# sh-lee97/grafx

Hardware: AMD Instinct MI355X
Metric: audio samples/sec (rendered output frames of the 32-channel console graph, all GPUs) (higher is better)
Workload: dtype f32; 1 GPU; BASELINE configs[3]: 32-channel mixing console, 111 nodes / 142 edges, ParametricEqualizer(6) + Compressor(iir) + STFTMaskedNoiseReverb + bus sums; batch_per_gpu=256, global_batch=256, audio_len=131072, channels=2, fsm_fir_len=4001, iir_len=16383, ir_len=60001, mode=forward render, reference-exact lengths (even L+N-1), parallelism=batch-shard x1, console_variant=headline, launch=eager render loop

## Files before the change

### grafx_amd/_lib.py

```python
import ctypes
import os

from .build import LIB

i64, f32p, vp, sz = ctypes.c_int64, ctypes.c_void_p, ctypes.c_void_p, ctypes.c_size_t


class RowMap(ctypes.Structure):
    _fields_ = [("inner", i64), ("stride_outer", i64), ("stride_inner", i64), ("stride_ch", i64)]


SIGNATURES = {
    "gfx_abi_version": (ctypes.c_int, []),
    "gfx_device_info": (ctypes.c_int, [ctypes.POINTER(ctypes.c_int), ctypes.POINTER(sz)]),
    "gfx_fftconv_nparts": (i64, [i64]),
    "gfx_fir_spectrum_bytes": (sz, [i64, i64]),
    "gfx_fftconv_workspace_bytes": (sz, [i64, i64, i64, i64, i64, i64]),
    "gfx_fir_spectrum_f32": (ctypes.c_int, [f32p, f32p, i64, vp, i64, i64, vp]),
    "gfx_fftconv_f32": (ctypes.c_int, [f32p, RowMap, vp, f32p, RowMap, i64, i64, i64, i64, i64, i64, i64, vp, sz, vp]),
    "gfx_fftconv_ex_f32": (ctypes.c_int, [f32p, RowMap, vp, i64, i64, f32p, RowMap, f32p, RowMap, i64, i64, i64, i64, i64, i64, i64, vp, sz, vp]),
    "gfx_fftconv_sched_f32": (ctypes.c_int, [f32p, RowMap, vp, i64, i64, f32p, RowMap, f32p, RowMap, i64, i64, i64, i64, i64, i64, i64, vp, sz, ctypes.c_int, vp]),
    "gfx_fftconv_rowmax_f32": (ctypes.c_int, [f32p, RowMap, vp, i64, i64, f32p, RowMap, f32p, RowMap, i64, i64, i64, i64, i64, i64, i64, vp, sz, vp, ctypes.POINTER(ctypes.c_int), vp]),
    "gfx_fftconv_state_f32": (ctypes.c_int, [f32p, RowMap, vp, i64, f32p, RowMap, f32p, f32p, i64, i64, i64, i64, i64, vp, sz,
                                             ctypes.c_int, vp]),
# ... 28 lines not shown
    "gfx_onepole_energy_f32": (ctypes.c_int, [f32p, RowMap, i64, f32p, f32p, i64, i64, i64, i64, ctypes.c_int, vp, vp]),
    "gfx_odd_alias_pair_rows_max_f32": (ctypes.c_int, [f32p, f32p, RowMap, i64, i64, i64, i64, i64, i64, vp, vp, sz, vp, vp]),
    "gfx_odd_alias_pair_precise_plan_bytes": (sz, [i64]),
    "gfx_odd_alias_pair_precise_workspace_bytes": (sz, [i64, i64]),
    "gfx_odd_alias_pair_precise_plan_f32": (ctypes.c_int, [vp, i64, vp, sz, vp]),
    "gfx_odd_alias_pair_precise_f32": (ctypes.c_int, [f32p, f32p, i64, i64, i64, i64, i64, vp, vp, sz, vp]),
    "gfx_irdft_f32": (ctypes.c_int, [f32p, ctypes.c_int, f32p, i64, i64, i64, i64, f32p, vp]),
    "gfx_rdft_f32": (ctypes.c_int, [f32p, f32p, i64, i64, i64, vp]),
    "gfx_iir_fsm_native": (ctypes.c_int, [i64]),
    "gfx_iir_fsm_plan_bytes": (sz, [i64]),
    "gfx_iir_fsm_plan_f32": (ctypes.c_int, [vp, i64, vp]),
    "gfx_iir_fsm_fir_f32": (ctypes.c_int, [f32p, f32p, vp, f32p, i64, i64, i64, vp]),
    "gfx_iir_fsm_fir_f64c_f32": (ctypes.c_int, [vp, vp, vp, f32p, i64, i64, i64, vp]),
    "gfx_iir_fsm_bwd_f32": (ctypes.c_int, [f32p, f32p, f32p, f32p, f32p, f32p, i64, i64, i64, vp]),
    "gfx_peq_coeffs_f32": (ctypes.c_int, [f32p, f32p, f32p, f32p, f32p, i64, i64, ctypes.c_int, vp]),
    "gfx_peq_coeffs_bwd_f32": (ctypes.c_int, [f32p] * 8 + [i64, i64, ctypes.c_int, vp]),
    "gfx_biquad_coeffs_f32": (ctypes.c_int, [f32p, f32p, f32p, f32p, f32p, f32p, i64, vp]),
    "gfx_dynamics_fused_f32": (ctypes.c_int, [f32p, RowMap, f32p, RowMap, f32p, f32p, f32p, f32p, i64, i64, i64,
                                              ctypes.c_int, i64, ctypes.c_int, ctypes.c_int, vp]),
    "gfx_dynamics_fused_ex_f32": (ctypes.c_int, [f32p, RowMap, f32p, RowMap, f32p, f32p, f32p, f32p, i64, i64, i64, i64,
                                                 ctypes.c_int, i64, ctypes.c_int, ctypes.c_int, vp]),
    "gfx_dynamics_fused_u1_f32": (ctypes.c_int, [f32p, RowMap, f32p, RowMap, f32p, f32p, f32p, f32p, i64, i64, i64, i64,
                                                 ctypes.c_int, i64, ctypes.c_int, ctypes.c_int, f32p, vp]),
    "gfx_dynamics_bwd_u1_f32": (ctypes.c_int, [f32p, RowMap, f32p, RowMap, f32p, f32p, f32p, f32p, i64, i64, i64, i64,
                                               ctypes.c_int, ctypes.c_int, f32p, RowMap, f32p, f32p, f32p, vp]),
    "gfx_dynamics_bwd_u1_ws_f32": (ctypes.c_int, [f32p, RowMap, f32p, RowMap, f32p, f32p, f32p, f32p, i64, i64, i64, i64,
                                                  ctypes.c_int, ctypes.c_int, f32p, RowMap, f32p, f32p, f32p, vp, sz, vp]),
    "gfx_dynamics_bwd_rescan_ws_f32": (ctypes.c_int, [f32p, RowMap, f32p, RowMap, f32p, f32p, f32p, f32p, i64, i64, i64, i64,
                                                      ctypes.c_int, ctypes.c_int, f32p, RowMap, f32p, f32p, f32p, vp, sz, vp]),
    "gfx_stft_f32": (ctypes.c_int, [f32p, f32p, f32p, i64, i64, i64, i64, vp]),
    "gfx_dynamics_ws_bytes": (sz, [i64]),
# ... 94 lines not shown
```

### grafx_amd/csrc/fft_tile.hpp

```cpp
#pragma once
#include <hip/hip_runtime.h>

namespace gfx {

constexpr int TILE_M = 8192;
constexpr int TILE_F = 16384;
constexpr int TILE_T = 256;
constexpr int S1_ROW = 272;
constexpr int S2_ROW = 18;
constexpr int TILE_LDS_F2 = 512 * S2_ROW;
constexpr int TILE_LDS_BYTES = TILE_LDS_F2 * 8;
constexpr int H_SLOTS = 17;
constexpr int H_TILE_F4 = H_SLOTS * TILE_T;

using cx = float __attribute__((ext_vector_type(2)));
using f4v = float __attribute__((ext_vector_type(4)));

__device__ __forceinline__ cx to_cx(float2 a) { return cx{a.x, a.y}; }
__device__ __forceinline__ cx cadd(cx a, cx b) { return a + b; }
__device__ __forceinline__ cx csub(cx a, cx b) { return a - b; }
__device__ __forceinline__ cx cswap(cx a) { return __builtin_shufflevector(a, a, 1, 0); }
__device__ __forceinline__ cx cconj(cx a) { return a * cx{1.0f, -1.0f}; }
__device__ __forceinline__ cx mul_neg_i(cx a) { return cswap(a) * cx{1.0f, -1.0f}; }
__device__ __forceinline__ cx mul_pos_i(cx a) { return cswap(a) * cx{-1.0f, 1.0f}; }
// ... 288 lines not shown
__device__ __forceinline__ void for_each_pair(int t, cx wj, Fn&& fn) {
    if (t != 0) {
#pragma unroll
        for (int k3 = 0; k3 < 16; ++k3) fn(k3, k3, 16 + (15 - k3), mul_w16(wj, k3), false);
    } else {
        const cx one = {1.0f, 0.0f};
        fn(0, 0, 0, one, true);
        fn(8, 8, 8, mul_w16(one, 8), true);
#pragma unroll
        for (int k3 = 1; k3 < 8; ++k3) fn(k3, k3, 16 - k3, mul_w16(one, k3), false);
#pragma unroll
        for (int k3 = 0; k3 < 8; ++k3) fn(9 + k3, 16 + k3, 16 + (15 - k3), tw32<false>(one, 1 + 2 * k3), false);
    }
}

}
```

### grafx_amd/csrc/fftconv.hip

```cpp
#include <hip/hip_runtime.h>

#include <cstdint>
#include <type_traits>

#include "../../include/grafx_amd.h"
#include "fft_tile.hpp"

namespace gfx {

struct ConvGeom {
    int64_t nparts, part_len, O, V, ntiles, hop;
    bool ok;
};

static inline ConvGeom conv_geom(int64_t N, int64_t Lout, int64_t part_len = 0) {
    ConvGeom g;
    g.ok = true;
    if (N <= TILE_M + 1) {
        g.nparts = 1;
        g.part_len = N;
        g.O = (N - 1 + 511) & ~int64_t(511);
        g.ok = part_len == 0;
    } else if (part_len == 0 || part_len == TILE_M) {
        g.part_len = TILE_M;
// ... 188 lines not shown

template <bool REV>
__global__ __launch_bounds__(TILE_T, 2) void hspec_kernel(const float* __restrict__ h, const float* __restrict__ gain,
                                                          int64_t gain_div, float4* __restrict__ Hs, int64_t N,
                                                          int nparts, int64_t part_len, gfx_rowmap_t hmap, int C,
                                                          const float2* __restrict__ twtab) {
    extern __shared__ __attribute__((aligned(16))) cx lds[];
    const int t = threadIdx.x;
    const unsigned b = blockIdx.x;
    const unsigned rc = b / (unsigned)nparts;
    const int p = (int)(b - rc * (unsigned)nparts);
    const int64_t start = (int64_t)p * part_len;
    const int64_t len = min(part_len, N - start);

    TileTw tw;
    cx v[32], w[2][16];
    if (REV) {
        const unsigned r = rc / (unsigned)C;
        load_window_rev(v, h + row_off(hmap, r, (int)(rc - r * (unsigned)C)) + (N - start - len), len, t);
    } else {
        load_window(v, h + (int64_t)rc * N + start, 0, len, t, gain ? gain[rc / (unsigned)gain_div] : 1.0f);
    }
    tile_twiddles(tw, twtab, t);
    tile_forward(v, w, tw, lds, t);

    f4v* out = reinterpret_cast<f4v*>(Hs) + (int64_t)b * H_TILE_F4;
    const float sc = 1.0f / (4.0f * TILE_M);
    for_each_pair(t, tw.base(), [&](int slot, int ia, int ib, cx, bool) {
        cx he, ho;
        pair_split(NAT(w, ia), NAT(w, ib), he, ho);
        out[slot * TILE_T + t] = __builtin_shufflevector(he * sc, ho * sc, 0, 1, 2, 3);
    });
}

__device__ __forceinline__ bool window_live(int64_t s, int64_t L) { return s + TILE_F > 0 && s < L; }

#define FC_STATE 0
#include "fftconv_window_kernels.hpp"
#undef FC_STATE
#define FC_STATE 1
#include "fftconv_window_kernels.hpp"
#undef FC_STATE

__global__ __launch_bounds__(TILE_T, 2) void macinv_kernel(const float2* __restrict__ Zs, const float4* __restrict__ Hs,
                                                           float* __restrict__ y, ConvArgs a, int64_t nwin,
                                                           const float2* __restrict__ twtab,
                                                           uint32_t* __restrict__ rowmax = nullptr) {
// ... 736 lines not shown
```

### grafx_amd/csrc/iir_fsm.hip

```cpp
#include <hip/hip_runtime.h>

#include <cstdint>

#include "../../include/grafx_amd.h"
#include "fft_tile.hpp"

#define NAT(arr, i) arr[(i) >> 4][brev((i) & 15, 4)]

namespace gfx {

constexpr int FSM_MAX_N = 4096;
constexpr int PLAN_CHIRP = TILE_M, PLAN_D = TILE_M + FSM_MAX_N, PLAN_FLOAT2 = PLAN_D + 2 * (FSM_MAX_N / 2 + 4);
static inline bool fsm_pow2(int64_t N) { return N == 8192 || N == 16384; }

__device__ __forceinline__ float2 chirp(int k, int N, float sign) {
    const int r = (int)(((int64_t)k * k) % (2 * (int64_t)N));
    float s, c;
    sincospif((float)r / (float)N, &s, &c);
    return make_float2(c, sign * s);
}

__device__ __forceinline__ void sample_points(int k, int N, float2& d1, float2& d2);

__global__ __launch_bounds__(TILE_T, 2) void bluestein_plan_kernel(float2* __restrict__ plan, int N,
// ... 62 lines not shown
                                                   float2 d1, float2 d2, int k, int N, const double* __restrict__ Bd = nullptr,
                                                   const double* __restrict__ Ad = nullptr) {
    if (Bd) return cascade_response_f64(Bd, Ad, K, k, N);
    float2 H = make_float2(1.0f, 0.0f);
    for (int i = 0; i < K; ++i) {
        const float b0 = B[3 * i], b1 = B[3 * i + 1], b2 = B[3 * i + 2];
        const float a0 = A[3 * i], a1 = A[3 * i + 1], a2 = A[3 * i + 2];
        const float2 num = make_float2((b0 + b1 * d1.x) + b2 * d2.x, (b1 * d1.y) + b2 * d2.y);
        const float2 den = make_float2((a0 + a1 * d1.x) + a2 * d2.x, (a1 * d1.y) + a2 * d2.y);
        const float2 q = cdiv(num, den);
        H = (i == 0) ? q : make_float2(fmaf(H.x, q.x, -H.y * q.y), fmaf(H.x, q.y, H.y * q.x));
    }
    return H;
}

__global__ __launch_bounds__(TILE_T, 2) void iir_fsm_kernel(const float* __restrict__ Bs, const float* __restrict__ As,
                                                            const float2* __restrict__ plan, float* __restrict__ h,
                                                            int K, int N, const float2* __restrict__ twtab,
                                                            const double* __restrict__ Bs64, const double* __restrict__ As64) {
    extern __shared__ __attribute__((aligned(16))) cx lds[];
    const int t = threadIdx.x;
    const int64_t rc = blockIdx.x;
    const float* B = Bs ? Bs + rc * K * 3 : nullptr;
    const float* A = As ? As + rc * K * 3 : nullptr;
    const double* Bd = Bs64 ? Bs64 + rc * K * 3 : nullptr;
    const double* Ad = As64 ? As64 + rc * K * 3 : nullptr;
    const int half = N / 2;
    const bool even = (N & 1) == 0;

    TileTw tw;
    tile_twiddles(tw, twtab, t);
    cx v[32], w[2][16];
#pragma unroll
    for (int a = 0; a < 9; ++a) {
        const int k = t + 256 * a;
        if (k <= half) {
            const float4 d = reinterpret_cast<const float4*>(plan + PLAN_D)[k];
            lds[k] = to_cx(cascade_response(B, A, K, make_float2(d.x, d.y), make_float2(d.z, d.w), k, N, Bd, Ad));
        }
    }
    __syncthreads();
#pragma unroll
    for (int a = 0; a < 32; ++a) {
        const int k = t + 256 * a;
        cx e = {0.0f, 0.0f};
        if (a < 17 && k < N) {
            const bool upper = k > half;
            cx Hk = lds[upper ? N - k : k];
            if (upper) Hk.y = -Hk.y;
            if (k == 0 || (even && k == half)) Hk.y = 0.0f;
            e = cmul(Hk, to_cx(plan[PLAN_CHIRP + k]));
        }
        v[a] = e;
    }
    __syncthreads();
    tile_forward(v, w, tw, lds, t);
#pragma unroll
    for (int q = 0; q < 32; ++q) w[q >> 4][q & 15] = cmul(w[q >> 4][q & 15], reinterpret_cast<const cx*>(plan)[q * TILE_T + t]);
    __syncthreads();
    tile_inverse(w, v, tw, lds, t);
    const float sc = 1.0f / ((float)N * (float)TILE_M);
    float* out = h + rc * N;
#pragma unroll
    for (int a = 0; a < 32; ++a) {
        const int n = t + 256 * a;
        if (n < N) {
            const float2 c = plan[PLAN_CHIRP + n];
            const cx e = v[brev(a, 5)];
            out[n] = (e.x * c.x - e.y * c.y) * sc;
        }
    }
}

__global__ __launch_bounds__(TILE_T, 2) void iir_fsm_pow2_kernel(const float* __restrict__ Bs, const float* __restrict__ As,
                                                                 float* __restrict__ h, int K, int N,
                                                                 const float2* __restrict__ twtab,
                                                                 const double* __restrict__ Bs64,
                                                                 const double* __restrict__ As64) {
    extern __shared__ __attribute__((aligned(16))) cx lds[];
    const int t = threadIdx.x;
    const int64_t rc = blockIdx.x;
    const float* B = Bs ? Bs + rc * K * 3 : nullptr;
    const float* A = As ? As + rc * K * 3 : nullptr;
    const double* Bd = Bs64 ? Bs64 + rc * K * 3 : nullptr;
    const double* Ad = As64 ? As64 + rc * K * 3 : nullptr;
    const int stride = TILE_F / N;
    TileTw tw;
    tile_twiddles(tw, twtab, t);
    cx v[32], w[2][16];
    auto Y = [&](int bin) -> cx {
        if (bin % stride) return cx{0.0f, 0.0f};
        const int k = bin / stride;
        float2 d1, d2;
        sample_points(k, N, d1, d2);
        cx r = to_cx(cascade_response(B, A, K, d1, d2, k, N, Bd, Ad));
        if (k == 0 || k == N / 2) r.y = 0.0f;
        return r;
    };
    for_each_pair(t, tw.base(), [&](int, int ia, int ib, cx, bool self) {
        const int j = (ia >> 4) ? bf_b(t) : bf_a(t);
        const int k = j + 512 * (ia & 15);
        const cx ya = Y(k), yb = (self && k != 0) ? ya : Y(TILE_M - k);
        float sn, cs;
        sincospif((float)k / (float)TILE_M, &sn, &cs);
        const cx ye = (ya + cconj(yb)) * 0.5f;
        const cx yo = cmul((ya - cconj(yb)) * 0.5f, cx{cs, sn});
        cx za, zb;
        pair_merge(ye, yo, za, zb);
        NAT(w, ia) = za;
        if (!self) NAT(w, ib) = zb;
    });
    tile_inverse(w, v, tw, lds, t);
    const float sc = (float)stride / (float)TILE_M;
    float* out = h + rc * N;
#pragma unroll
    for (int a = 0; a < 32; ++a) {
        const int n = 2 * (t + 256 * a);
        const cx e = v[brev(a, 5)] * sc;
        if (n + 1 < N) *reinterpret_cast<float2*>(out + n) = make_float2(e.x, e.y);
    }
}

__global__ void peq_coeffs_kernel(const float* __restrict__ w0, const float* __restrict__ q_inv,
                                  const float* __restrict__ log_gain, float* __restrict__ Bs, float* __restrict__ As,
                                  int64_t n, int K, int shelving) {
    const int64_t i = (int64_t)blockIdx.x * blockDim.x + threadIdx.x;
    if (i >= n * K) return;
    const int band = (int)(i % K);
    const float pi32 = 3.14159274101257324219f;
    const float w = pi32 * (1.0f / (1.0f + expf(-w0[i])));
    const float qi = expf(q_inv[i]);
    const float A = expf(log_gain[i]);
    float sw, cw;
    sincosf(w, &sw, &cw);
    const float alpha = sw * qi * 0.5f;
    float b0, b1, b2, a0, a1, a2;
    const bool low = shelving && band == 0, high = shelving && band == K - 1;
    if (low || high) {
        const float sg = low ? 1.0f : -1.0f;
        const float ap1 = A + 1.0f, am1 = A - 1.0f;
        const float ap1c = ap1 * cw, am1c = am1 * cw;
        const float s = 2.0f * sqrtf(A) * alpha;
        b0 = A * ((ap1 - sg * am1c) + s);
        b1 = sg * 2.0f * A * (am1 - sg * ap1c);
        b2 = A * ((ap1 - sg * am1c) - s);
        a0 = (ap1 + sg * am1c) + s;
        a1 = -sg * 2.0f * (am1 + sg * ap1c);
        a2 = (ap1 + sg * am1c) - s;
    } else {
        const float aA = alpha * A, adA = alpha / A;
        b0 = 1.0f + aA;
        b1 = -2.0f * cw;
        b2 = 1.0f - aA;
        a0 = 1.0f + adA;
        a1 = b1;
        a2 = 1.0f - adA;
    }
    Bs[3 * i] = b0;
    Bs[3 * i + 1] = b1;
    Bs[3 * i + 2] = b2;
    As[3 * i] = a0;
    As[3 * i + 1] = a1;
    As[3 * i + 2] = a2;
}

__global__ void peq_coeffs_bwd_kernel(const float* __restrict__ w0, const float* __restrict__ q_inv,
                                      const float* __restrict__ log_gain, const float* __restrict__ gBs,
                                      const float* __restrict__ gAs, float* __restrict__ gw0, float* __restrict__ gq,
                                      float* __restrict__ glg, int64_t n, int K, int shelving) {
    const int64_t i = (int64_t)blockIdx.x * blockDim.x + threadIdx.x;
    if (i >= n * K) return;
    const int band = (int)(i % K);
    const float pi32 = 3.14159274101257324219f;
    const float sig = 1.0f / (1.0f + expf(-w0[i]));
    const float w = pi32 * sig;
    const float qi = expf(q_inv[i]);
    const float A = expf(log_gain[i]);
    float sw, cw;
// ... 155 lines not shown
int gfx_iir_fsm_fir_f64c_f32(const double* Bs, const double* As, const void* plan, float* h, int64_t RC, int64_t K,
                             int64_t N, void* stream) {
    if (!Bs || !As) return GFX_EINVAL;
    return iir_fsm_fir_launch(nullptr, nullptr, Bs, As, plan, h, RC, K, N, stream);
}

int gfx_peq_coeffs_f32(const float* w0, const float* q_inv, const float* log_gain, float* Bs, float* As, int64_t n,
                       int64_t K, int use_shelving, void* stream) {
    if (!w0 || !q_inv || !log_gain || !Bs || !As || n <= 0 || K <= 0) return GFX_EINVAL;
    const int64_t total = n * K;
    hipLaunchKernelGGL(peq_coeffs_kernel, dim3((unsigned)((total + 255) / 256)), dim3(256), 0, (hipStream_t)stream, w0,
                       q_inv, log_gain, Bs, As, n, (int)K, use_shelving);
    return hipGetLastError() == hipSuccess ? GFX_OK : GFX_ELAUNCH;
}

int gfx_peq_coeffs_bwd_f32(const float* w0, const float* q_inv, const float* log_gain, const float* gBs, const float* gAs,
                           float* gw0, float* gq_inv, float* glog_gain, int64_t n, int64_t K, int use_shelving,
                           void* stream) {
    if (!w0 || !q_inv || !log_gain || !gBs || !gAs || !gw0 || !gq_inv || !glog_gain || n <= 0 || K <= 0) return GFX_EINVAL;
    const int64_t total = n * K;
    hipLaunchKernelGGL(peq_coeffs_bwd_kernel, dim3((unsigned)((total + 255) / 256)), dim3(256), 0, (hipStream_t)stream, w0,
                       q_inv, log_gain, gBs, gAs, gw0, gq_inv, glog_gain, n, (int)K, use_shelving);
    return hipGetLastError() == hipSuccess ? GFX_OK : GFX_ELAUNCH;
}

int gfx_biquad_coeffs_f32(const float* Bin, const float* A1_pre, const float* A2_pre, const float* A0, float* Bs,
                          float* As, int64_t n, void* stream) {
    if (!Bin || !A1_pre || !A2_pre || !Bs || !As || n <= 0) return GFX_EINVAL;
    hipLaunchKernelGGL(biquad_coeffs_kernel, dim3((unsigned)((n + 255) / 256)), dim3(256), 0, (hipStream_t)stream, Bin,
                       A1_pre, A2_pre, A0, Bs, As, n);
// ... 15 lines not shown
```

### grafx_amd/ops.py

```python
import contextvars
import ctypes
import os

import torch

from ._lib import RowMap, check, lib


_PROFILE = contextvars.ContextVar("grafx_amd_profile", default=None)


class profiling:
    def __enter__(self):
        self.record = {}
        self.token = _PROFILE.set(self.record)
        return self.record

    def __exit__(self, *exc):
        _PROFILE.reset(self.token)
        return False


class _timed:
    def __init__(self, name, nbytes):
# ... 532 lines not shown


@_on_device
def peq_coeffs(w0, q_inv, log_gain, use_shelving=True):
    _require_gpu(w0, q_inv, log_gain)
    w0, q_inv, log_gain = w0.contiguous(), q_inv.contiguous(), log_gain.contiguous()
    K = w0.shape[-1]
    n = w0.numel() // K
    Bs = torch.empty((*w0.shape, 3), dtype=torch.float32, device=w0.device)
    As = torch.empty_like(Bs)
    check(lib().gfx_peq_coeffs_f32(_ptr(w0), _ptr(q_inv), _ptr(log_gain), _ptr(Bs), _ptr(As), n, K, int(use_shelving), _stream()),
          "gfx_peq_coeffs_f32")
    return Bs, As


@_on_device
def peq_coeffs_bwd(w0, q_inv, log_gain, gBs, gAs, use_shelving=True):
    _require_gpu(w0, q_inv, log_gain, gBs, gAs)
    w0, q_inv, log_gain = w0.contiguous(), q_inv.contiguous(), log_gain.contiguous()
    _expect(gBs, (*w0.shape, 3), "peq_coeffs_bwd: gBs")
    _expect(gAs, (*w0.shape, 3), "peq_coeffs_bwd: gAs")
    K = w0.shape[-1]
    out = [torch.empty_like(w0) for _ in range(3)]
    pin = _Pin()
    check(lib().gfx_peq_coeffs_bwd_f32(_ptr(w0), _ptr(q_inv), _ptr(log_gain), pin(gBs), pin(gAs),
                                       *(_ptr(o) for o in out), w0.numel() // K, K, int(use_shelving), _stream()),
          "gfx_peq_coeffs_bwd_f32")
    return tuple(out)


# ... 653 lines not shown
```

### grafx_amd/processors/core/iir.py

```python
import torch
import torch.nn as nn

from ... import autograd as diff
from ... import ops
from ...autograd import needs_grad
from ._buffer_io import StreamIO, write_rows
from .convolution import FIRConvolution, check_state, convolve_taps


def map_signal(fn, result):
    return (fn(result[0]), *result[1:]) if isinstance(result, tuple) else fn(result)


class BiquadStream(StreamIO):

    def stream_block(self, x4, out4, carry, **params):
        key = "history" if self.biquad.backend == "fsm" else "state"
        y, carry = self.forward(x4.reshape(-1, *x4.shape[2:]), **params, **{key: carry, "return_" + key: True})
        write_rows(out4, y)
        return carry


class IIRFilter(nn.Module):
    def __init__(self, order=2, backend="fsm", flashfftconv=True, fsm_fir_len=4000,
# ... 134 lines not shown
        if needs_grad(x, Bs, As, history):
            if N <= self.FSM_NATIVE_MAX and Bs.shape[-1] == 3:
                h = diff.FsmFirFn.apply(Bs, As, N, self._plan(Bs.device))
            else:
                h = diff.fsm_fir(Bs, As, N)
            y, zf = diff.convolve(x, h, "causal", final=final, state=check_state(history, x, N, "IIRFilter(backend='fsm')"),
                                  return_state=True)
            if out is not None:
                out.copy_(y.view(out.shape))
                y = out
        else:
            y, zf = convolve_taps(x, ops.fir_spectrum(self._taps(Bs, As)), N, Bs.shape[1], "causal", out=out,
                                  h_rows=shared_rows, state=history, return_state=True)
        return (y, zf) if return_history else y

    def forward(self, input_signal, Bs, As, out=None, tee=None, shared_rows=None, final=False, state=None,
                return_state=False, history=None, return_history=False):
        if self.backend == "fsm" and (state is not None or return_state):
            raise ValueError("IIRFilter(backend='fsm'): the frequency-sampled FIR carries no recursive state; use the "
                             "recursive backends (backend='lfilter' or 'ssm') for block-wise processing")
        if history is not None or return_history:
            if self.backend != "fsm":
                raise ValueError(f"IIRFilter(backend={self.backend!r}): history / return_history carry the input history of the "
                                 "frequency-sampled FIR (backend='fsm'); a recursive backend carries state / return_state")
            return self._process_fsm_block(input_signal, Bs, As, out, tee, shared_rows, final, history, return_history)
        if shared_rows is not None and self.backend != "fsm":
            rows = input_signal.shape[0] * input_signal.shape[1] if input_signal.ndim == 4 else input_signal.shape[0]
            Bs, As = Bs.repeat(rows // shared_rows, 1, 1, 1), As.repeat(rows // shared_rows, 1, 1, 1)
            shared_rows = None
        if self.backend != "fsm":
# ... 22 lines not shown
```

### grafx_amd/processors/eq.py

```python
import torch
import torch.nn as nn

from .. import ops
from .core._buffer_io import BufferIO, Prepared, StreamIO, expand_shared, shared_reps, write_rows
from .core.convolution import convolve, convolve_taps
from .core.fir import ZeroPhaseFilterBankFIR, ZeroPhaseFIR
from .core.geq import GraphicEqualizerBiquad
from .. import autograd as diff
from ..autograd import needs_grad
from .core.iir import BiquadStream, IIRFilter, map_signal
from .core.midside import lr_to_ms, ms_to_lr


class ParametricEqualizer(BufferIO, nn.Module):
    def __init__(self, num_filters=10, processor_channel="mono", use_shelving_filters=True, **backend_kwargs):
        super().__init__()
        self.num_filters = num_filters
        self.use_shelving_filters = use_shelving_filters
        self.biquad = IIRFilter(order=2, **backend_kwargs)
        self.processor_channel = processor_channel
        if processor_channel not in ("mono", "stereo", "midside"):
            raise ValueError(f"Invalid processor_channel: {self.processor_channel}")

    accepts_tee = True
    accepts_shared_params = True
    accepts_strided_rows = True

    def forward(self, input_signals, w0, q_inv, log_gain, _out=None, _tee=None, _shared_rows=None, state=None,
                return_state=False, history=None, return_history=False):
        self._check_bands()
        if needs_grad(input_signals, w0, q_inv, log_gain):
            Bs, As = diff.PeqCoeffsFn.apply(w0, q_inv, log_gain, self.use_shelving_filters)
        else:
            Bs, As = ops.peq_coeffs(w0, q_inv, log_gain, self.use_shelving_filters)
        block = {} if state is None and not return_state else {"state": state, "return_state": return_state}
        if history is not None or return_history:
            block.update(history=history, return_history=return_history)
        if self.processor_channel == "midside":
            y = self.biquad(lr_to_ms(input_signals), Bs, As, shared_rows=_shared_rows, final=True, **block)
            return (ms_to_lr(y[0]), y[1]) if return_state or return_history else ms_to_lr(y)
        return self.biquad(input_signals, Bs, As, out=_out, tee=_tee, shared_rows=_shared_rows, final=True, **block)

    def get_biquad_coefficients_with_shelving_filters(self, cos_w0, alpha, A):
        from .filter import HighShelf, LowShelf, PeakingFilter

        self._check_bands()
        K = self.num_filters
        parts = [LowShelf.get_biquad_coefficients(cos_w0[..., :1], alpha[..., :1], A[..., :1]),
                 PeakingFilter.get_biquad_coefficients(cos_w0[..., 1 : K - 1], alpha[..., 1 : K - 1], A[..., 1 : K - 1]),
                 HighShelf.get_biquad_coefficients(cos_w0[..., K - 1 :], alpha[..., K - 1 :], A[..., K - 1 :])]
        return torch.cat([b for b, _ in parts], -2), torch.cat([a for _, a in parts], -2)

    def _check_bands(self):
        if self.use_shelving_filters and self.num_filters < 2:
            raise RuntimeError(f"split expects non-negative sizes, got [1, {self.num_filters - 2}, 1]: "
                               "shelving filters need num_filters >= 2")

    def prepare(self, w0, q_inv, log_gain, _shared_rows=None):
        self._check_bands()
        if self.processor_channel == "midside" or self.biquad.backend != "fsm" or needs_grad(w0, q_inv, log_gain):
            return None
        Bs, As = ops.peq_coeffs(w0, q_inv, log_gain, self.use_shelving_filters)
        return Prepared(ops.fir_spectrum(self.biquad._taps(Bs, As)), Cf=Bs.shape[1])

    def render_into(self, x4, out4, tee=None, _shared_rows=None, _prepared=None, history=None, return_history=False,
                    **params):
        if history is not None or return_history:
            if _prepared is not None:
                y, zf = convolve_taps(x4, _prepared.tensors[0], self.biquad.fsm_fir_len, _prepared.Cf, "causal", out=out4,
                                      tee=tee, h_rows=_shared_rows, state=history, return_state=True)
            elif self.processor_channel == "midside":
                if tee is not None:
                    tee.copy_(x4)
                y, zf = self.forward(x4, _shared_rows=_shared_rows, history=history, return_history=True, **params)
                y = write_rows(out4, y)
            else:
                y, zf = self.forward(x4, _out=out4, _tee=tee, _shared_rows=_shared_rows, history=history,
                                     return_history=True, **params)
# ... 97 lines not shown
```

### grafx_amd/render/graph.py

```python
import contextlib
import warnings

import torch

from ..data.configs import UTILITY_TYPES
from .core import (
    aggregate_tensor,
    create_signal_buffer,
    expand_tensor_or_tensor_dict,
    flatten_batch_and_node,
    inplace_write_tensor,
    read_tensor_or_tensor_dict,
)


KEEP_SMOOTHER_SCAN = False
PREPARE_MODE = "under_first"

BLOCK_FAN_ADJOINT = True


def _gather_plan(step, device):
    cache = step.__dict__.setdefault("_plans", {})
    key = (device.type, device.index)
# ... 245 lines not shown
                      keep_signal_buffer=True):
    from .. import ops

    squeeze = input_signals.ndim == 3
    x = input_signals.unsqueeze(0) if squeeze else input_signals
    B, n_src, C, L = x.shape
    shared_tree = per_type_parameters if (not squeeze and common_parameters is None) else None
    if not squeeze:
        expanded_tree = None
        if common_parameters is not None:
            common_parameters = expand_tensor_or_tensor_dict(common_parameters, expand=B, dim=0)
    node_dim = 0 if squeeze else 1
    postprocess = None if squeeze else flatten_batch_and_node

    buf = torch.empty(B, render_data.num_nodes, C, L, device=x.device)
    lean = not keep_signal_buffer
    teed = None if lean else _tee_range(render_data, processors, n_src, x.device)
    main = torch.cuda.current_stream(x.device)
    rest = [] if lean else _complement(teed, n_src)
    sources_in_buf = not lean
    side = _side_stream(x.device) if rest else None
    if side is not None:
        side.wait_stream(main)
        with torch.cuda.stream(side):
            for a, b in rest:
                buf[:, a:b].copy_(x[:, a:b], non_blocking=True)
    copied = False
    out_view = None

    def ensure_sources():
        nonlocal sources_in_buf
        if not sources_in_buf:
            buf[:, :n_src].copy_(x)
            sources_in_buf = True

    def stage_parameters(step, proc):
        nonlocal expanded_tree
        extra = {}
        if squeeze:
            params = read_tensor_or_tensor_dict(per_type_parameters[step.node_type], step.parameter_read, dim=0)
        elif shared_tree is not None and getattr(proc, "accepts_shared_params", False):
            params = read_tensor_or_tensor_dict(shared_tree[step.node_type], step.parameter_read, dim=0)
            extra["_shared_rows"] = step.dest_write.idx[1] - step.dest_write.idx[0]
        else:
# ... 18 lines not shown
        prep.wait_stream(main)
        ready = {}
        with torch.cuda.stream(prep):
            for j in todo:
                proc_j = processors[render_data.iter_list[j].node_type]
                extra_j, params_j, common_j = args[j]
                state = proc_j.prepare(**extra_j, **params_j, **common_j)
                if state is None:
                    continue
                for tns in state.tensors:
                    tns.record_stream(main)
                event = torch.cuda.Event()
                event.record(prep)
                ready[j] = (state, event)
        return ready

    prepared = None
    launched = 0
    done = set()

    def run_stage(i, mix_with=None):
        nonlocal copied, prepared, launched
        step = render_data.iter_list[i]
        d0, d1 = step.dest_write.idx
        out_v = buf.narrow(1, d0, d1 - d0)
        plan = _gather_plan(step, x.device)
        node_type = step.node_type
        src_read = step.source_reads[0]
        from_inputs = plan is None and src_read.idx[1] <= n_src
        if side is not None and not from_inputs and not copied and _touches_inputs(src_read, n_src):
# ... 2 lines not shown
        if lean and not from_inputs and _touches_inputs(src_read, n_src):
            ensure_sources()
        if node_type not in processors:
            if plan is None:
                a, b = step.source_reads[0].idx
                out_v.copy_((x if from_inputs else buf).narrow(1, a, b - a))
            else:
                _gather(ops, buf, plan, out_v)
            return False
        if plan is None:
            a, b = step.source_reads[0].idx
            x_view = (x if from_inputs else buf).narrow(1, a, b - a)
        else:
            x_view = _gather(ops, buf, plan, torch.empty(B, plan[2], C, L, device=x.device))
        proc = processors[node_type]
        extra, params, common_i = stage_parameters(step, proc)
        if teed is not None and i == _first_order(render_data):
            a, b = teed
            extra["tee"] = buf.narrow(1, a, b - a)
        if prepared is not None and i in prepared:
            state, event = prepared[i]
            main.wait_event(event)
            extra["_prepared"] = state
        if (aux is not None and plan is None and KEEP_SMOOTHER_SCAN and getattr(proc, "accepts_aux", False)
                and type(proc) in _tape_safe_types()):
            extra["_aux"] = (aux, i)
        mix = None
        if mix_with is not None:
            nxt = render_data.iter_list[mix_with]
            sched = _mix_schedule(step, nxt, x.device)
            if side is not None and not copied and any(r < n_src for r in sched["extra_rows"]):
# ... 646 lines not shown
```

### include/grafx_amd.h

```cpp
#ifndef GRAFX_AMD_H
#define GRAFX_AMD_H

#include <stddef.h>
#include <stdint.h>

#ifdef __cplusplus
extern "C" {
#endif

#define GFX_OK 0
#define GFX_EINVAL -1
#define GFX_ENOSPC -2
#define GFX_ELAUNCH -3

typedef struct {
    int64_t inner;
    int64_t stride_outer;
    int64_t stride_inner;
    int64_t stride_ch;
} gfx_rowmap_t;

int gfx_abi_version(void);
int gfx_device_info(int* n_cu, size_t* lds_bytes);

// ... 92 lines not shown

int gfx_iir_fsm_native(int64_t N);
size_t gfx_iir_fsm_plan_bytes(int64_t N);
int gfx_iir_fsm_plan_f32(void* plan, int64_t N, void* stream);
int gfx_iir_fsm_fir_f32(const float* Bs, const float* As, const void* plan, float* h,
                        int64_t RC, int64_t K, int64_t N, void* stream);
int gfx_iir_fsm_fir_f64c_f32(const double* Bs, const double* As, const void* plan, float* h, int64_t RC, int64_t K,
                             int64_t N, void* stream);
int gfx_iir_fsm_bwd_f32(const float* Bs, const float* As, const float* G, const float* delays, float* gB, float* gA,
                        int64_t RC, int64_t K, int64_t N, void* stream);

int gfx_peq_coeffs_f32(const float* w0, const float* q_inv, const float* log_gain, float* Bs, float* As,
                       int64_t n, int64_t K, int use_shelving, void* stream);
int gfx_biquad_coeffs_f32(const float* Bin, const float* A1_pre, const float* A2_pre, const float* A0,
                          float* Bs, float* As, int64_t n, void* stream);
int gfx_peq_coeffs_bwd_f32(const float* w0, const float* q_inv, const float* log_gain, const float* gBs,
                           const float* gAs, float* gw0, float* gq_inv, float* glog_gain,
                           int64_t n, int64_t K, int use_shelving, void* stream);

int gfx_dynamics_fused_f32(const float* x, gfx_rowmap_t xmap, float* y, gfx_rowmap_t ymap,
                           const float* log_threshold, const float* log_ratio, const float* log_knee,
                           const float* z_alpha, int64_t R, int64_t C, int64_t L, int smoother,
                           int64_t iir_len, int knee, int gate, void* stream);
int gfx_dynamics_fused_ex_f32(const float* x, gfx_rowmap_t xmap, float* y, gfx_rowmap_t ymap,
                              const float* log_threshold, const float* log_ratio, const float* log_knee,
                              const float* z_alpha, int64_t param_rows, int64_t R, int64_t C, int64_t L,
                              int smoother, int64_t iir_len, int knee, int gate, void* stream);
size_t gfx_dynamics_ws_bytes(int64_t param_rows);
size_t gfx_dynamics_ws_bytes_ex(int64_t param_rows, int64_t R, int64_t L);
int gfx_dynamics_fused_ws_f32(const float* x, gfx_rowmap_t xmap, float* y, gfx_rowmap_t ymap,
// ... 155 lines not shown
```

Baseline: 3.366 billion audio samples/s.

## Fuse PEQ coefficient design, FSM impulse response, and filter spectrum into one kernel

Adds a peq_spectra kernel that computes biquad coefficients in LDS, evaluates the frequency-sampled IIR response, and directly produces the tiled FIR spectrum, replacing three separate launches (peq_coeffs, iir_fsm taps, fir_spectrum) and their intermediate global buffers. The render loop also prepares the first-order stage's design before the source copy setup so it can overlap. Shared device helpers are factored out of the existing FSM and spectrum kernels. This adds a large-register, LDS-heavy kernel with one block per row, which could occupy the GPU less efficiently than the separate kernels.

```diff
diff --git a/grafx_amd/_lib.py b/grafx_amd/_lib.py
--- a/grafx_amd/_lib.py
+++ b/grafx_amd/_lib.py
@@ -66,7 +66,8 @@
     "gfx_iir_fsm_fir_f64c_f32": (ctypes.c_int, [vp, vp, vp, f32p, i64, i64, i64, vp]),
     "gfx_iir_fsm_bwd_f32": (ctypes.c_int, [f32p, f32p, f32p, f32p, f32p, f32p, i64, i64, i64, vp]),
     "gfx_peq_coeffs_f32": (ctypes.c_int, [f32p, f32p, f32p, f32p, f32p, i64, i64, ctypes.c_int, vp]),
-    "gfx_peq_coeffs_bwd_f32": (ctypes.c_int, [f32p] * 8 + [i64, i64, ctypes.c_int, vp]),
+    "gfx_peq_spectra_f32": (ctypes.c_int, [f32p, f32p, f32p, RowMap, vp, vp, i64, i64, i64, i64, ctypes.c_int, vp]),
+    "gfx_peq_coeffs_bwd_f32":(ctypes.c_int, [f32p] * 8 + [i64, i64, ctypes.c_int, vp]),
     "gfx_biquad_coeffs_f32": (ctypes.c_int, [f32p, f32p, f32p, f32p, f32p, f32p, i64, vp]),
     "gfx_dynamics_fused_f32": (ctypes.c_int, [f32p, RowMap, f32p, RowMap, f32p, f32p, f32p, f32p, i64, i64, i64,
                                               ctypes.c_int, i64, ctypes.c_int, ctypes.c_int, vp]),
diff --git a/grafx_amd/csrc/fft_tile.hpp b/grafx_amd/csrc/fft_tile.hpp
--- a/grafx_amd/csrc/fft_tile.hpp
+++ b/grafx_amd/csrc/fft_tile.hpp
@@ -326,4 +326,15 @@
     }
 }
 
-}
+__device__ __forceinline__ void tile_filter_spectrum(cx (&v)[32], const TileTw& tw, cx* lds, int t, f4v* __restrict__ out) {
+    cx w[2][16];
+    tile_forward(v, w, tw, lds, t);
+    const float sc = 1.0f / (4.0f * TILE_M);
+    for_each_pair(t, tw.base(), [&](int slot, int ia, int ib, cx, bool) {
+        cx he, ho;
+        pair_split(w[ia >> 4][brev(ia & 15, 4)], w[ib >> 4][brev(ib & 15, 4)], he, ho);
+        out[slot * TILE_T + t] = __builtin_shufflevector(he * sc, ho * sc, 0, 1, 2, 3);
+    });
+}
+
+}
diff --git a/grafx_amd/csrc/fftconv.hip b/grafx_amd/csrc/fftconv.hip
--- a/grafx_amd/csrc/fftconv.hip
+++ b/grafx_amd/csrc/fftconv.hip
@@ -226,7 +226,7 @@
     const int64_t len = min(part_len, N - start);
 
     TileTw tw;
-    cx v[32], w[2][16];
+    cx v[32];
     if (REV) {
         const unsigned r = rc / (unsigned)C;
         load_window_rev(v, h + row_off(hmap, r, (int)(rc - r * (unsigned)C)) + (N - start - len), len, t);
@@ -234,15 +234,7 @@
         load_window(v, h + (int64_t)rc * N + start, 0, len, t, gain ? gain[rc / (unsigned)gain_div] : 1.0f);
     }
     tile_twiddles(tw, twtab, t);
-    tile_forward(v, w, tw, lds, t);
-
-    f4v* out = reinterpret_cast<f4v*>(Hs) + (int64_t)b * H_TILE_F4;
-    const float sc = 1.0f / (4.0f * TILE_M);
-    for_each_pair(t, tw.base(), [&](int slot, int ia, int ib, cx, bool) {
-        cx he, ho;
-        pair_split(NAT(w, ia), NAT(w, ib), he, ho);
-        out[slot * TILE_T + t] = __builtin_shufflevector(he * sc, ho * sc, 0, 1, 2, 3);
-    });
+    tile_filter_spectrum(v, tw, lds, t, reinterpret_cast<f4v*>(Hs) + (int64_t)b * H_TILE_F4);
 }
 
 __device__ __forceinline__ bool window_live(int64_t s, int64_t L) { return s + TILE_F > 0 && s < L; }
diff --git a/grafx_amd/csrc/iir_fsm.hip b/grafx_amd/csrc/iir_fsm.hip
--- a/grafx_amd/csrc/iir_fsm.hip
+++ b/grafx_amd/csrc/iir_fsm.hip
@@ -100,6 +100,49 @@
     return H;
 }
 
+constexpr int FSM_COEF_AT = FSM_MAX_N;
+constexpr int FSM_COEF_MAX_K = 1024;
+__device__ __forceinline__ void fsm_czt(const float* __restrict__ B, const float* __restrict__ A, const double* __restrict__ Bd,
+                                        const double* __restrict__ Ad, const float2* __restrict__ plan, int K, int N,
+                                        const TileTw& tw, cx* lds, int t, cx (&v)[32]) {
+    const int half = N / 2;
+    const bool even = (N & 1) == 0;
+    cx w[2][16];
+#pragma unroll
+    for (int a = 0; a < 9; ++a) {
+        const int k = t + 256 * a;
+        if (k <= half) {
+            const float4 d = reinterpret_cast<const float4*>(plan + PLAN_D)[k];
+            lds[k] = to_cx(cascade_response(B, A, K, make_float2(d.x, d.y), make_float2(d.z, d.w), k, N, Bd, Ad));
+        }
+    }
+    __syncthreads();
+#pragma unroll
+    for (int a = 0; a < 32; ++a) {
+        const int k = t + 256 * a;
+        cx e = {0.0f, 0.0f};
+        if (a < 17 && k < N) {
+            const bool upper = k > half;
+            cx Hk = lds[upper ? N - k : k];
+            if (upper) Hk.y = -Hk.y;
+            if (k == 0 || (even && k == half)) Hk.y = 0.0f;
+            e = cmul(Hk, to_cx(plan[PLAN_CHIRP + k]));
+        }
+        v[a] = e;
+    }
+    __syncthreads();
+    tile_forward(v, w, tw, lds, t);
+#pragma unroll
+    for (int q = 0; q < 32; ++q) w[q >> 4][q & 15] = cmul(w[q >> 4][q & 15], reinterpret_cast<const cx*>(plan)[q * TILE_T + t]);
+    __syncthreads();
+    tile_inverse(w, v, tw, lds, t);
+}
+__device__ __forceinline__ float fsm_tap(const cx (&v)[32], const float2* __restrict__ plan, int a, int n, float sc) {
+    const float2 c = plan[PLAN_CHIRP + n];
+    const cx e = v[brev(a, 5)];
+    return (e.x * c.x - e.y * c.y) * sc;
+}
+
 __global__ __launch_bounds__(TILE_T, 2) void iir_fsm_kernel(const float* __restrict__ Bs, const float* __restrict__ As,
                                                             const float2* __restrict__ plan, float* __restrict__ h,
                                                             int K, int N, const float2* __restrict__ twtab,
@@ -111,69 +154,24 @@
     const float* A = As ? As + rc * K * 3 : nullptr;
     const double* Bd = Bs64 ? Bs64 + rc * K * 3 : nullptr;
     const double* Ad = As64 ? As64 + rc * K * 3 : nullptr;
-    const int half = N / 2;
-    const bool even = (N & 1) == 0;
-
     TileTw tw;
     tile_twiddles(tw, twtab, t);
-    cx v[32], w[2][16];
-#pragma unroll
-    for (int a = 0; a < 9; ++a) {
-        const int k = t + 256 * a;
-        if (k <= half) {
-            const float4 d = reinterpret_cast<const float4*>(plan + PLAN_D)[k];
-            lds[k] = to_cx(cascade_response(B, A, K, make_float2(d.x, d.y), make_float2(d.z, d.w), k, N, Bd, Ad));
-        }
-    }
-    __syncthreads();
-#pragma unroll
-    for (int a = 0; a < 32; ++a) {
-        const int k = t + 256 * a;
-        cx e = {0.0f, 0.0f};
-        if (a < 17 && k < N) {
-            const bool upper = k > half;
-            cx Hk = lds[upper ? N - k : k];
-            if (upper) Hk.y = -Hk.y;
-            if (k == 0 || (even && k == half)) Hk.y = 0.0f;
-            e = cmul(Hk, to_cx(plan[PLAN_CHIRP + k]));
-        }
-        v[a] = e;
-    }
-    __syncthreads();
-    tile_forward(v, w, tw, lds, t);
-#pragma unroll
-    for (int q = 0; q < 32; ++q) w[q >> 4][q & 15] = cmul(w[q >> 4][q & 15], reinterpret_cast<const cx*>(plan)[q * TILE_T + t]);
-    __syncthreads();
-    tile_inverse(w, v, tw, lds, t);
+    cx v[32];
+    fsm_czt(B, A, Bd, Ad, plan, K, N, tw, lds, t, v);
     const float sc = 1.0f / ((float)N * (float)TILE_M);
     float* out = h + rc * N;
 #pragma unroll
     for (int a = 0; a < 32; ++a) {
         const int n = t + 256 * a;
-        if (n < N) {
-            const float2 c = plan[PLAN_CHIRP + n];
-            const cx e = v[brev(a, 5)];
-            out[n] = (e.x * c.x - e.y * c.y) * sc;
-        }
-    }
-}
-
-__global__ __launch_bounds__(TILE_T, 2) void iir_fsm_pow2_kernel(const float* __restrict__ Bs, const float* __restrict__ As,
-                                                                 float* __restrict__ h, int K, int N,
-                                                                 const float2* __restrict__ twtab,
-                                                                 const double* __restrict__ Bs64,
-                                                                 const double* __restrict__ As64) {
-    extern __shared__ __attribute__((aligned(16))) cx lds[];
-    const int t = threadIdx.x;
-    const int64_t rc = blockIdx.x;
-    const float* B = Bs ? Bs + rc * K * 3 : nullptr;
-    const float* A = As ? As + rc * K * 3 : nullptr;
-    const double* Bd = Bs64 ? Bs64 + rc * K * 3 : nullptr;
-    const double* Ad = As64 ? As64 + rc * K * 3 : nullptr;
+        if (n < N) out[n] = fsm_tap(v, plan, a, n, sc);
+    }
+}
+
+__device__ __forceinline__ float fsm_pow2_scale(int N) { return (float)(TILE_F / N) / (float)TILE_M; }
+__device__ __forceinline__ void fsm_pow2_spectrum(const float* __restrict__ B, const float* __restrict__ A,
+                                                  const double* __restrict__ Bd, const double* __restrict__ Ad, int K, int N,
+                                                  const TileTw& tw, int t, cx (&w)[2][16]) {
     const int stride = TILE_F / N;
-    TileTw tw;
-    tile_twiddles(tw, twtab, t);
-    cx v[32], w[2][16];
     auto Y = [&](int bin) -> cx {
         if (bin % stride) return cx{0.0f, 0.0f};
         const int k = bin / stride;
@@ -196,8 +194,26 @@
         NAT(w, ia) = za;
         if (!self) NAT(w, ib) = zb;
     });
+}
+
+__global__ __launch_bounds__(TILE_T, 2) void iir_fsm_pow2_kernel(const float* __restrict__ Bs, const float* __restrict__ As,
+                                                                 float* __restrict__ h, int K, int N,
+                                                                 const float2* __restrict__ twtab,
+                                                                 const double* __restrict__ Bs64,
+                                                                 const double* __restrict__ As64) {
+    extern __shared__ __attribute__((aligned(16))) cx lds[];
+    const int t = threadIdx.x;
+    const int64_t rc = blockIdx.x;
+    const float* B = Bs ? Bs + rc * K * 3 : nullptr;
+    const float* A = As ? As + rc * K * 3 : nullptr;
+    const double* Bd = Bs64 ? Bs64 + rc * K * 3 : nullptr;
+    const double* Ad = As64 ? As64 + rc * K * 3 : nullptr;
+    TileTw tw;
+    tile_twiddles(tw, twtab, t);
+    cx v[32], w[2][16];
+    fsm_pow2_spectrum(B, A, Bd, Ad, K, N, tw, t, w);
     tile_inverse(w, v, tw, lds, t);
-    const float sc = (float)stride / (float)TILE_M;
+    const float sc = fsm_pow2_scale(N);
     float* out = h + rc * N;
 #pragma unroll
     for (int a = 0; a < 32; ++a) {
@@ -207,16 +223,12 @@
     }
 }
 
-__global__ void peq_coeffs_kernel(const float* __restrict__ w0, const float* __restrict__ q_inv,
-                                  const float* __restrict__ log_gain, float* __restrict__ Bs, float* __restrict__ As,
-                                  int64_t n, int K, int shelving) {
-    const int64_t i = (int64_t)blockIdx.x * blockDim.x + threadIdx.x;
-    if (i >= n * K) return;
-    const int band = (int)(i % K);
+__device__ __forceinline__ void peq_section(float w0, float q_inv, float log_gain, int band, int K, int shelving,
+                                            float* __restrict__ Bs, float* __restrict__ As) {
     const float pi32 = 3.14159274101257324219f;
-    const float w = pi32 * (1.0f / (1.0f + expf(-w0[i])));
-    const float qi = expf(q_inv[i]);
-    const float A = expf(log_gain[i]);
+    const float w = pi32 * (1.0f / (1.0f + expf(-w0)));
+    const float qi = expf(q_inv);
+    const float A = expf(log_gain);
     float sw, cw;
     sincosf(w, &sw, &cw);
     const float alpha = sw * qi * 0.5f;
@@ -242,12 +254,80 @@
         a1 = b1;
         a2 = 1.0f - adA;
     }
-    Bs[3 * i] = b0;
-    Bs[3 * i + 1] = b1;
-    Bs[3 * i + 2] = b2;
-    As[3 * i] = a0;
-    As[3 * i + 1] = a1;
-    As[3 * i + 2] = a2;
+    Bs[0] = b0;
+    Bs[1] = b1;
+    Bs[2] = b2;
+    As[0] = a0;
+    As[1] = a1;
+    As[2] = a2;
+}
+
+__global__ void peq_coeffs_kernel(const float* __restrict__ w0, const float* __restrict__ q_inv,
+                                  const float* __restrict__ log_gain, float* __restrict__ Bs, float* __restrict__ As,
+                                  int64_t n, int K, int shelving) {
+    const int64_t i = (int64_t)blockIdx.x * blockDim.x + threadIdx.x;
+    if (i >= n * K) return;
+    peq_section(w0[i], q_inv[i], log_gain[i], (int)(i % K), K, shelving, Bs + 3 * i, As + 3 * i);
+}
+
+template <bool POW2>
+__global__ __launch_bounds__(TILE_T, 2) void peq_spectra_kernel(const float* __restrict__ w0, const float* __restrict__ q_inv,
+                                                                const float* __restrict__ log_gain, gfx_rowmap_t pmap, int Cf,
+                                                                const float2* __restrict__ plan, float4* __restrict__ Hs,
+                                                                int K, int N, int shelving,
+                                                                const float2* __restrict__ twtab) {
+    extern __shared__ __attribute__((aligned(16))) cx lds[];
+    const int t = threadIdx.x;
+    const unsigned rc = blockIdx.x;
+    const unsigned r = rc / (unsigned)Cf;
+    const int c = (int)(rc - r * (unsigned)Cf);
+    const unsigned q = r / (unsigned)pmap.inner;
+    const int64_t p0 = (int64_t)q * pmap.stride_outer + (int64_t)(r - q * (unsigned)pmap.inner) * pmap.stride_inner +
+                       (int64_t)c * pmap.stride_ch;
+    float* B = reinterpret_cast<float*>(lds + FSM_COEF_AT);
+    float* A = B + 3 * K;
+    for (int band = t; band < K; band += TILE_T)
+        peq_section(w0[p0 + band], q_inv[p0 + band], log_gain[p0 + band], band, K, shelving, B + 3 * band, A + 3 * band);
+    __syncthreads();
+
+    TileTw tw;
+    tile_twiddles(tw, twtab, t);
+    cx v[32], h2[32];
+    if (POW2) {
+        cx w[2][16];
+        fsm_pow2_spectrum(B, A, nullptr, nullptr, K, N, tw, t, w);
+        __syncthreads();
+        tile_inverse(w, v, tw, lds, t);
+        const float sc = fsm_pow2_scale(N);
+#pragma unroll
+        for (int a = 0; a < 32; ++a) {
+            const cx e = v[brev(a, 5)] * sc;
+            h2[a] = 2 * (t + 256 * a) + 1 < N ? e : cx{0.0f, 0.0f};
+        }
+    } else {
+        fsm_czt(B, A, nullptr, nullptr, plan, K, N, tw, lds, t, v);
+        const float sc = 1.0f / ((float)N * (float)TILE_M);
+        float* taps = reinterpret_cast<float*>(lds);
+        __syncthreads();
+#pragma unroll
+        for (int a = 0; a < FSM_MAX_N / TILE_T; ++a) {
+            const int n = t + 256 * a;
+            if (n < N) taps[n] = fsm_tap(v, plan, a, n, sc);
+        }
+        __syncthreads();
+#pragma unroll
+        for (int a = 0; a < 32; ++a) {
+            const int n = 2 * (t + 256 * a);
+            cx e = {0.0f, 0.0f};
+            if (a < FSM_MAX_N / 2 / TILE_T) {
+                if (n < N) e.x = taps[n];
+                if (n + 1 < N) e.y = taps[n + 1];
+            }
+            h2[a] = e;
+        }
+    }
+    __syncthreads();
+    tile_filter_spectrum(h2, tw, lds, t, reinterpret_cast<f4v*>(Hs) + (int64_t)rc * H_TILE_F4);
 }
 
 __global__ void peq_coeffs_bwd_kernel(const float* __restrict__ w0, const float* __restrict__ q_inv,
@@ -433,6 +513,21 @@
     return hipGetLastError() == hipSuccess ? GFX_OK : GFX_ELAUNCH;
 }
 
+int gfx_peq_spectra_f32(const float* w0, const float* q_inv, const float* log_gain, gfx_rowmap_t pmap, const void* plan,
+                        void* Hs, int64_t R, int64_t Cf, int64_t K, int64_t N, int use_shelving, void* stream) {
+    if (!w0 || !q_inv || !log_gain || !Hs || R <= 0 || Cf <= 0 || K <= 0 || K > FSM_COEF_MAX_K) return GFX_EINVAL;
+    if (pmap.inner <= 0 || pmap.inner > 0x7fffffffLL || R * Cf > 0x7fffffffLL) return GFX_EINVAL;
+    const bool pow2 = N == TILE_M;
+    if (!pow2 && (N < 1 || N > FSM_MAX_N || !plan)) return GFX_EINVAL;
+    auto* kernel = pow2 ? peq_spectra_kernel<true> : peq_spectra_kernel<false>;
+    if (allow_lds(kernel)) return GFX_ELAUNCH;
+    const float2* tw = tile_twiddle_table((hipStream_t)stream);
+    if (!tw) return GFX_ELAUNCH;
+    hipLaunchKernelGGL(kernel, dim3((unsigned)(R * Cf)), dim3(TILE_T), TILE_LDS_BYTES, (hipStream_t)stream, w0, q_inv,
+                       log_gain, pmap, (int)Cf, (const float2*)plan, (float4*)Hs, (int)K, (int)N, use_shelving, tw);
+    return hipGetLastError() == hipSuccess ? GFX_OK : GFX_ELAUNCH;
+}
+
 int gfx_peq_coeffs_bwd_f32(const float* w0, const float* q_inv, const float* log_gain, const float* gBs, const float* gAs,
                            float* gw0, float* gq_inv, float* glog_gain, int64_t n, int64_t K, int use_shelving,
                            void* stream) {
diff --git a/grafx_amd/ops.py b/grafx_amd/ops.py
--- a/grafx_amd/ops.py
+++ b/grafx_amd/ops.py
@@ -570,6 +570,31 @@
     return Bs, As
 
 
+PEQ_SPECTRA_MAX_K = 1024
+
+
+def peq_spectra_native(N, K):
+    return 1 <= K <= PEQ_SPECTRA_MAX_K and (1 <= N <= 4096 or N == 8192)
+
+
+@_on_device
+def peq_spectra(w0, q_inv, log_gain, N, plan, use_shelving=True):
+    _require_gpu(w0, q_inv, log_gain)
+    if w0.ndim != 3:
+        raise ValueError(f"peq_spectra: expected (R, Cf, K) parameters, got {tuple(w0.shape)}")
+    _expect(q_inv, w0.shape, "peq_spectra: q_inv")
+    _expect(log_gain, w0.shape, "peq_spectra: log_gain")
+    if w0.stride(-1) != 1 or q_inv.stride() != w0.stride() or log_gain.stride() != w0.stride():
+        w0, q_inv, log_gain = w0.contiguous(), q_inv.contiguous(), log_gain.contiguous()
+    R, Cf, K = w0.shape
+    nbytes = lib().gfx_fir_spectrum_bytes_ex(R * Cf, N, 0) if peq_spectra_native(N, K) else 0
+    Hs = torch.empty(nbytes, dtype=torch.uint8, device=w0.device)
+    pmap = RowMap(max(R, 1), 0, w0.stride(0), w0.stride(1))
+    check(lib().gfx_peq_spectra_f32(_ptr(w0), _ptr(q_inv), _ptr(log_gain), pmap, _ptr(plan), _ptr(Hs), R, Cf, K, N,
+                                    int(use_shelving), _stream()), "gfx_peq_spectra_f32")
+    return Hs
+
+
 @_on_device
 def peq_coeffs_bwd(w0, q_inv, log_gain, gBs, gAs, use_shelving=True):
     _require_gpu(w0, q_inv, log_gain, gBs, gAs)
diff --git a/grafx_amd/processors/core/iir.py b/grafx_amd/processors/core/iir.py
--- a/grafx_amd/processors/core/iir.py
+++ b/grafx_amd/processors/core/iir.py
@@ -172,6 +172,14 @@
                                   h_rows=shared_rows, state=history, return_state=True)
         return (y, zf) if return_history else y
 
+    def convolve_spectra(self, x, Hs, Cf, out=None, tee=None, shared_rows=None, history=None, return_history=False):
+        N = self.fsm_fir_len
+        if history is not None or return_history:
+            y, zf = convolve_taps(x, Hs, N, Cf, "causal", out=out, tee=tee, h_rows=shared_rows, state=history,
+                                  return_state=True)
+            return (y, zf) if return_history else y
+        return convolve_taps(x, Hs, N, Cf, "causal", out=out, tee=tee, exact=self.flashfftconv, h_rows=shared_rows)
+
     def forward(self, input_signal, Bs, As, out=None, tee=None, shared_rows=None, final=False, state=None,
                 return_state=False, history=None, return_history=False):
         if self.backend == "fsm" and (state is not None or return_state):
diff --git a/grafx_amd/processors/eq.py b/grafx_amd/processors/eq.py
--- a/grafx_amd/processors/eq.py
+++ b/grafx_amd/processors/eq.py
@@ -29,6 +29,10 @@
     def forward(self, input_signals, w0, q_inv, log_gain, _out=None, _tee=None, _shared_rows=None, state=None,
                 return_state=False, history=None, return_history=False):
         self._check_bands()
+        if state is None and not return_state and self._designs_fused(input_signals, w0, q_inv, log_gain):
+            return self.biquad.convolve_spectra(input_signals, self._design(w0, q_inv, log_gain), w0.shape[1], out=_out,
+                                                tee=_tee, shared_rows=_shared_rows, history=history,
+                                                return_history=return_history)
         if needs_grad(input_signals, w0, q_inv, log_gain):
             Bs, As = diff.PeqCoeffsFn.apply(w0, q_inv, log_gain, self.use_shelving_filters)
         else:
@@ -51,6 +55,18 @@
                  HighShelf.get_biquad_coefficients(cos_w0[..., K - 1 :], alpha[..., K - 1 :], A[..., K - 1 :])]
         return torch.cat([b for b, _ in parts], -2), torch.cat([a for _, a in parts], -2)
 
+    def _designs_fused(self, *tensors):
+        w0 = tensors[-3]
+        return (self.biquad.backend == "fsm" and self.processor_channel != "midside" and not needs_grad(*tensors)
+                and w0.ndim == 3 and ops.peq_spectra_native(self.biquad.fsm_fir_len, w0.shape[-1]))
+
+    def _design(self, w0, q_inv, log_gain):
+        if self._designs_fused(w0, q_inv, log_gain):
+            plan = self.biquad._plan(w0.device) if w0.is_cuda else None
+            return ops.peq_spectra(w0, q_inv, log_gain, self.biquad.fsm_fir_len, plan, self.use_shelving_filters)
+        Bs, As = ops.peq_coeffs(w0, q_inv, log_gain, self.use_shelving_filters)
+        return ops.fir_spectrum(self.biquad._taps(Bs, As))
+
     def _check_bands(self):
         if self.use_shelving_filters and self.num_filters < 2:
             raise RuntimeError(f"split expects non-negative sizes, got [1, {self.num_filters - 2}, 1]: "
@@ -60,8 +76,7 @@
         self._check_bands()
         if self.processor_channel == "midside" or self.biquad.backend != "fsm" or needs_grad(w0, q_inv, log_gain):
             return None
-        Bs, As = ops.peq_coeffs(w0, q_inv, log_gain, self.use_shelving_filters)
-        return Prepared(ops.fir_spectrum(self.biquad._taps(Bs, As)), Cf=Bs.shape[1])
+        return Prepared(self._design(w0, q_inv, log_gain), Cf=w0.shape[1])
 
     def render_into(self, x4, out4, tee=None, _shared_rows=None, _prepared=None, history=None, return_history=False,
                     **params):
diff --git a/grafx_amd/render/graph.py b/grafx_amd/render/graph.py
--- a/grafx_amd/render/graph.py
+++ b/grafx_amd/render/graph.py
@@ -283,20 +283,6 @@
     postprocess = None if squeeze else flatten_batch_and_node
 
     buf = torch.empty(B, render_data.num_nodes, C, L, device=x.device)
-    lean = not keep_signal_buffer
-    teed = None if lean else _tee_range(render_data, processors, n_src, x.device)
-    main = torch.cuda.current_stream(x.device)
-    rest = [] if lean else _complement(teed, n_src)
-    sources_in_buf = not lean
-    side = _side_stream(x.device) if rest else None
-    if side is not None:
-        side.wait_stream(main)
-        with torch.cuda.stream(side):
-            for a, b in rest:
-                buf[:, a:b].copy_(x[:, a:b], non_blocking=True)
-    copied = False
-    out_view = None
-
     def ensure_sources():
         nonlocal sources_in_buf
         if not sources_in_buf:
@@ -345,6 +331,28 @@
                 event.record(prep)
                 ready[j] = (state, event)
         return ready
+
+    first_args = first_design = None
+    if PREPARE_MODE != "inline" and render_data.max_order >= 1:
+        step1 = render_data.iter_list[_first_order(render_data)]
+        proc1 = processors[step1.node_type] if step1.node_type in processors else None
+        if hasattr(proc1, "prepare"):
+            first_args = stage_parameters(step1, proc1)
+            first_design = proc1.prepare(**first_args[0], **first_args[1], **first_args[2])
+
+    lean = not keep_signal_buffer
+    teed = None if lean else _tee_range(render_data, processors, n_src, x.device)
+    main = torch.cuda.current_stream(x.device)
+    rest = [] if lean else _complement(teed, n_src)
+    sources_in_buf = not lean
+    side = _side_stream(x.device) if rest else None
+    if side is not None:
+        side.wait_stream(main)
+        with torch.cuda.stream(side):
+            for a, b in rest:
+                buf[:, a:b].copy_(x[:, a:b], non_blocking=True)
+    copied = False
+    out_view = None
 
     prepared = None
     launched = 0
@@ -377,7 +385,12 @@
         else:
             x_view = _gather(ops, buf, plan, torch.empty(B, plan[2], C, L, device=x.device))
         proc = processors[node_type]
-        extra, params, common_i = stage_parameters(step, proc)
+        if first_args is not None and i == _first_order(render_data):
+            extra, params, common_i = first_args
+            if first_design is not None:
+                extra["_prepared"] = first_design
+        else:
+            extra, params, common_i = stage_parameters(step, proc)
         if teed is not None and i == _first_order(render_data):
             a, b = teed
             extra["tee"] = buf.narrow(1, a, b - a)
diff --git a/include/grafx_amd.h b/include/grafx_amd.h
--- a/include/grafx_amd.h
+++ b/include/grafx_amd.h
@@ -130,6 +130,8 @@
                        int64_t n, int64_t K, int use_shelving, void* stream);
 int gfx_biquad_coeffs_f32(const float* Bin, const float* A1_pre, const float* A2_pre, const float* A0,
                           float* Bs, float* As, int64_t n, void* stream);
+int gfx_peq_spectra_f32(const float* w0, const float* q_inv, const float* log_gain, gfx_rowmap_t pmap, const void* plan,
+                        void* Hs, int64_t R, int64_t Cf, int64_t K, int64_t N, int use_shelving, void* stream);
 int gfx_peq_coeffs_bwd_f32(const float* w0, const float* q_inv, const float* log_gain, const float* gBs,
                            const float* gAs, float* gw0, float* gq_inv, float* glog_gain,
                            int64_t n, int64_t K, int use_shelving, void* stream);
```

After: 3.372 billion audio samples/s (median of 4 runs). About the same (+0.2%).
